# kosmylo/Safe-MARL

Measured on AMD Instinct MI355X. Metric: env-steps/sec (33-bus, 4096 envs/GPU) at 1/2/4/8 MI355X + PF-kernel HBM GB/s, higher is better.
Workload: dtype f64

## Files before the change

safe-marl_amd/csrc/flexenv.hip:

```cpp
#include <hip/hip_runtime.h>
#include <stdint.h>
#include <stdio.h>
#include <string.h>
#include <stdlib.h>
#include <vector>
#include "flex_device.h"
#include "flexnet.h"
#include "actor_r16.h"
#include "agent_sum.h"

#define FLEX_MAX_DEVICES 16
#define HIP_TRY(x) do { hipError_t _e = (x); if (_e != hipSuccess) { \
    fprintf(stderr, "[flexenv] %s failed: %s (%s:%d)\n", #x, hipGetErrorString(_e), __FILE__, __LINE__); \
    return FLEX_EHIP; } } while (0)

enum { AF_E = 0, AF_PRED, AF_CH, AF_DIS, AF_Q, AF_PCT, AF_EINIT, AF_COUNT };
enum { IF_STEPS = 0, IF_START, IF_ROW, IF_OBSCNT, IF_ITERS, IF_SWEEPS, IF_EPISODE, IF_COUNT = 8 };
__host__ __device__ __forceinline__ int agent_rec_doubles(int n_agents) { return (AF_COUNT * n_agents + 7) & ~7; }

struct DevState {
    double* vm;
    uint32_t* vw;
    double* agent;
    double* cumrew;
// ... 172 lines not shown
            const bool live = NA_EXACT || ag < na;
#pragma unroll
            for (int i = 0; i < CLS; ++i) {
                const flex_v2i r = __builtin_amdgcn_raw_buffer_load_b64(rin, live ? src[i] : -1, ag * H3 * 16, 0);
                buf[ag][i] = make_float2(__int_as_float(r.x), __int_as_float(r.y));
            }
        }
    }
    __device__ __forceinline__ void store(const KArgs& a, int env0, bool enable, OutT* __restrict__ out) const {
        const int H = a.cfg.history, na = a.cfg.n_agents, H3 = 3 * H;
        const int env_floats = na * H * 6;
        const int span = enable ? EPW * env_floats : 0;
        const __amdgpu_buffer_rsrc_t rout = __builtin_amdgcn_make_buffer_rsrc(
            (void*)(out + (int64_t)env0 * env_floats), 0, span * (int)sizeof(OutT), FLEX_BUF_FLAGS);
#pragma unroll
        for (int ag = 0; ag < NA_CAP; ++ag) {
            const bool live = NA_EXACT || ag < na;
#pragma unroll
            for (int i = 0; i < CLS; ++i) {
                const int d = live ? dst[i] : -1;
                if constexpr (sizeof(OutT) == 4) {
                    flex_v2i w; w.x = __float_as_int(buf[ag][i].x); w.y = __float_as_int(buf[ag][i].y);
                    __builtin_amdgcn_raw_buffer_store_b64(w, rout, d, ag * H3 * 8, FLEX_AUX_NT);
                } else {
                    const double dx = (double)buf[ag][i].x, dy = (double)buf[ag][i].y;
                    flex_v4i w; w.x = __double2loint(dx); w.y = __double2hiint(dx); w.z = __double2loint(dy); w.w = __double2hiint(dy);
                    __builtin_amdgcn_raw_buffer_store_b128(w, rout, d, ag * H3 * 16, FLEX_AUX_NT);
                }
            }
        }
    }
};

template <int EPW, typename OutT>
__device__ __forceinline__ void obs_store_new(const KArgs& a, int env0, int g, bool valid, const LaneNet& ln, int k,
                                              double pd, double qd, double ppv, double v, double price, double e,
                                              OutT* __restrict__ out, float* __restrict__ rows) {
    const int H = a.cfg.history, na = a.cfg.n_agents;
    const int ring_floats = na * H * 12, env_floats = na * H * 6;
    float* const ring = a.st.ring + (int64_t)env0 * ring_floats;
    const int slot = small_mod(k, H, a.inv_h);
    if (valid && ln.agent >= 0) {
        const float2 r0 = make_float2((float)pd, (float)qd), r1 = make_float2((float)ppv, (float)v);
        const float2 r2 = make_float2((float)price, (float)e);
        const uint32_t ro = (uint32_t)(g * ring_floats + (ln.agent * 2 * H + slot) * 6) * 4, mo = ro + (uint32_t)H * 24;
        st_at2(ring, ro, r0); st_at2(ring, ro + 8, r1); st_at2(ring, ro + 16, r2);
        st_at2(ring, mo, r0); st_at2(ring, mo + 8, r1); st_at2(ring, mo + 16, r2);
        if (rows) {
            typedef float rw_f4 __attribute__((ext_vector_type(4)));
            float* const rb = rows + (int64_t)env0 * (na * FLEX_ROW_W);
            const uint32_t wo = (uint32_t)((g * na + ln.agent) * FLEX_ROW_W) * 4;
            const float older = (float)(k < H - 1 ? k : H - 1);
            st_at<rw_f4>(rb, wo, rw_f4{r0.x, r0.y, r1.x, r1.y});
            st_at<rw_f4>(rb, wo + 16, rw_f4{r2.x, r2.y, older, 0.0f});
        }
        if (out) {
            OutT* const o = out + (int64_t)env0 * env_floats;
            const uint32_t oo = (uint32_t)(g * env_floats + (ln.agent * H + (H - 1)) * 6) * (uint32_t)sizeof(OutT);
            if constexpr (sizeof(OutT) == 4) {
                st_at2(o, oo, r0); st_at2(o, oo + 8, r1); st_at2(o, oo + 16, r2);
            } else {
                st_at<double>(o, oo, pd); st_at<double>(o, oo + 8, qd); st_at<double>(o, oo + 16, ppv);
                st_at<double>(o, oo + 24, v); st_at<double>(o, oo + 32, price); st_at<double>(o, oo + 40, e);
            }
        }
    }
}

template <int EPW>
__device__ __forceinline__ void obs_ring_clear(const KArgs& a, int env, bool valid, const LaneNet& ln) {
    constexpr int LW = FLEX_WAVE / EPW;
    const int H = a.cfg.history, na = a.cfg.n_agents;
    float* ring = a.st.ring + (int64_t)env * na * H * 12;
    const int per_agent = (H - 1) * 6;
    if (valid)
        for (int idx = ln.l; idx < na * per_agent; idx += LW) {
            const int ag = idx / per_agent, rem = idx - ag * per_agent;
            ring[(ag * 2 * H + 1) * 6 + rem] = 0.0f;
        }
}

template <int EPW, typename OutT>
__device__ __forceinline__ void push_and_emit_obs(const KArgs& a, int env, bool valid, const LaneNet& ln, int k,
                                                  double pd, double qd, double ppv, double v, double price,
                                                  double e, OutT* __restrict__ out, float* __restrict__ rows, bool fresh) {
    constexpr int LW = FLEX_WAVE / EPW;
    const int H = a.cfg.history, na = a.cfg.n_agents;
    int32_t* ie = a.st.ienv + (int64_t)env * IF_COUNT;
    const int slot = k % H;
    float* ring = a.st.ring + (int64_t)env * na * H * 12;
    OutT* o = out ? out + (int64_t)env * na * H * 6 : nullptr;
    if (valid && ln.agent >= 0) {
        const double feat[6] = {pd, qd, ppv, v, price, e};
        float* r = ring + (ln.agent * 2 * H + slot) * 6;
#pragma unroll
        for (int t = 0; t < 6; ++t) {
            r[t] = (float)feat[t];
            r[H * 6 + t] = (float)feat[t];
            if (o) o[(ln.agent * H + (H - 1)) * 6 + t] = (OutT)feat[t];
// ... 119 lines not shown
        if (failed) { if (or_failed) { if (!ok) failed[env] = 1; } else failed[env] = ok ? 0 : 1; }
    }
    if (ln.l == FLEX_WAVE / EPW - 1 && valid) a.st.cumrew[env] = 0.0;
    obs_ring_clear<EPW>(a, env, valid, ln);
    if (want_obs) push_and_emit_obs<EPW, ObsT>(a, env, valid, ln, 0, pd, qd, ppv, v, price, e_new, obs, rows, true);
}

template <int EPW, typename ObsT>
__global__ __launch_bounds__(FLEX_WAVE * FLEX_WAVES_PER_BLOCK)
void flex_reset_kernel(KArgs a, const uint8_t* __restrict__ mask, DevResetSpec inj, ObsT* __restrict__ obs,
                       int want_obs, uint8_t* __restrict__ failed) {
    EnvSlot<EPW> slot(a.n_envs);
    if (slot.wave_idle(a.n_envs)) return;
    const bool valid = slot.valid && (!mask || mask[slot.env] != 0);
    if (__ballot(valid) == 0ull) return;
    LaneNet ln;
    load_lane_net<EPW>(a.net, slot.lane, ln);
    flex_reset_body<EPW, ObsT>(a, slot.env, valid, ln, inj, obs, want_obs, nullptr, failed, false);
}


#ifndef FLEX_MANY_CARRY_NET
#define FLEX_MANY_CARRY_NET 1
#endif
#ifndef FLEX_MANY_PREFETCH_ACT
#define FLEX_MANY_PREFETCH_ACT 1
#endif
#ifndef FLEX_MANY_EARLY_HEAD
#define FLEX_MANY_EARLY_HEAD 1
#endif
#ifndef FLEX_MANY_HDR_REGS
#define FLEX_MANY_HDR_REGS 1
#endif
struct StepCarry {
    flex_v4i iv;
    bool have;
    bool have_iv;
    LaneNet ln;
    NetHdrRegs hdr;
    float4 af;
    double2 ad0, ad1;
#ifdef FLEX_MANY_STAMPS
    uint32_t st_prev, st_acc[4];
#endif
    double pd, qd, ppv, price, e_cur, e_init, cum;
    uint32_t vw;
};
template <int EPW, typename ObsT, typename ActT, int NA_CAP, bool SINK, bool ROWS, bool MANY = false>
__device__ __forceinline__ void flex_step_body(const KArgs& a, const int wave, const ActT* __restrict__ actions,
                                               double* __restrict__ reward, uint8_t* __restrict__ done, double* __restrict__ info,
                                               uint8_t* __restrict__ failed, ObsT* __restrict__ obs, int want_obs, int auto_reset,
                                               const int64_t slab, const bool cells, const unsigned long long kbase,
                                               StepCarry* mc = nullptr, const ActT* __restrict__ next_actions = nullptr) {
    constexpr int LW = FLEX_WAVE / EPW;
    const int lane = threadIdx.x & 63;
    const int env0 = wave * EPW;
    if (env0 >= a.n_envs) return;
    float* rowrec = nullptr;
    if constexpr (ROWS) {
        if (a.obs_slabs > 0 && obs) {
            const int64_t p = (slab >= 0 ? slab : *a.obs_cursor) + 1;
            rowrec = reinterpret_cast<float*>(obs) + (p >= a.obs_slabs ? 0 : p) * a.obs_slab_stride;
        }
    }
    const bool valid = env0 + lane / LW < a.n_envs;
    const int g = valid ? lane / LW : 0;
    const int env = env0 + g;
    FLEX_STAMP_RT(5);
    FLEX_STAMP(0);
    const FlexCfg& c = a.cfg;
    int32_t* const b_ienv = a.st.ienv + (int64_t)env0 * IF_COUNT;
    const uint32_t o_ienv = g * (IF_COUNT * 4);
    int4 iv;
    LaneNet ln;
    if constexpr (MANY) {
        if (mc->have || mc->have_iv) iv = int4{mc->iv.x, mc->iv.y, mc->iv.z, mc->iv.w};
        else iv = ld_at<int4>(b_ienv, o_ienv);
#if FLEX_MANY_CARRY_NET
        ln = mc->ln;
#else
        load_lane_net<EPW>(a.net, lane, ln);
#endif
    } else {
        iv = ld_at<int4>(b_ienv, o_ienv);
        load_lane_net<EPW>(a.net, lane, ln);
    }
    ln.pq = ln.pq && valid;
    const int nb = a.n_bus, na = c.n_agents;
    const bool is_bus = ln.bus >= 0, is_bld = ln.agent >= 0;
    const int ag = is_bld ? ln.agent : 0, busi = is_bus ? ln.bus : 0;

    const int arec = agent_rec_doubles(na);
    double* const b_agent = a.st.agent + (int64_t)env0 * arec;
    uint32_t* const b_vw = a.st.vw + (int64_t)env0 * LW;
    const ActT* const b_act = actions + (int64_t)env0 * (na * 4);
    const uint32_t o_agent = (g * arec + ag) * 8;
    const uint32_t o_volt = (g * LW + ln.l) * 4;
    const uint32_t o_bus = busi * 8, o_qbus = (nb + busi) * 8, o_pv = (2 * nb + ag) * 8, o_price = (2 * nb + na) * 8;
    const uint32_t AFB = na * 8;

    const int steps = iv.x, start = iv.y, obs_cnt = iv.w;
    const int rows = (int)a.rows;
    const uint32_t row_off = (uint32_t)clamp_row32(iv.z, rows) * (uint32_t)a.row_bytes;

    const bool from_regs = MANY && mc->have;
    const uint32_t o_act = (g * na + ag) * (4 * (uint32_t)sizeof(ActT));
    ActT av[4];
    if constexpr (MANY && FLEX_MANY_PREFETCH_ACT) {
        if constexpr (sizeof(ActT) == 4) { av[0] = mc->af.x; av[1] = mc->af.y; av[2] = mc->af.z; av[3] = mc->af.w; }
        else { av[0] = mc->ad0.x; av[1] = mc->ad0.y; av[2] = mc->ad1.x; av[3] = mc->ad1.y; }
    } else if constexpr (sizeof(ActT) == 4) {
        const float4 t = ld_at<float4>(b_act, o_act);
        av[0] = t.x; av[1] = t.y; av[2] = t.z; av[3] = t.w;
    } else {
        const double2 t0 = ld_at<double2>(b_act, o_act), t1 = ld_at<double2>(b_act, o_act + 16);
        av[0] = t0.x; av[1] = t0.y; av[2] = t1.x; av[3] = t1.y;
    }
    double pd_r, qd_r, ppv_r, price, e_cur_r, e_init_r, cum_before;
    uint32_t vw_word;
    if (from_regs) {
        pd_r = mc->pd; qd_r = mc->qd; ppv_r = mc->ppv; price = mc->price;
        e_cur_r = mc->e_cur; e_init_r = mc->e_init; cum_before = mc->cum; vw_word = mc->vw;
    } else {
        pd_r = ld_at<double>(a.series, row_off + o_bus); qd_r = ld_at<double>(a.series, row_off + o_qbus);
        ppv_r = ld_at<double>(a.series, row_off + o_pv); price = ld_at<double>(a.series, row_off + o_price);
        e_cur_r = ld_at<double>(b_agent, o_agent + AF_E * AFB);
        e_init_r = ld_at<double>(b_agent, o_agent + AF_EINIT * AFB);
        vw_word = ld_at<uint32_t>(b_vw, o_volt);
        cum_before = ld_at<double>(a.st.cumrew + env0, g * 8);
    }
    double we, wf;
    unpack_warm(vw_word, we, wf);
    const int new_row = clamp_row32(start + steps, rows);
    const uint32_t nrow_off = (uint32_t)new_row * (uint32_t)a.row_bytes;
    if constexpr (MANY && FLEX_MANY_PREFETCH_ACT) {
        const ActT* const b_nact = next_actions + (int64_t)env0 * (na * 4);
        if constexpr (sizeof(ActT) == 4) mc->af = ld_at<float4>(b_nact, o_act);
        else { mc->ad0 = ld_at<double2>(b_nact, o_act); mc->ad1 = ld_at<double2>(b_nact, o_act + 16); }
    }
    double n_pd = ld_at<double>(a.series, nrow_off + (is_bld || MANY ? o_bus : o_price));
    double n_qd = ld_at<double>(a.series, nrow_off + (is_bld || MANY ? o_qbus : o_price));
    double n_ppv = ld_at<double>(a.series, nrow_off + (is_bld || MANY ? o_pv : o_price));
    const double n_price = ld_at<double>(a.series, nrow_off + o_price);
    const bool obs_fast = want_obs && (ROWS || (na <= NA_CAP && 3 * c.history <= FLEX_OBS_CLASSES(EPW) * LW));
    ObsHist<EPW, ROWS ? 1 : NA_CAP, ObsT> hist;
    if constexpr (!ROWS) hist.load(a, env0, g, valid, obs_fast, ln, obs_cnt);

    const bool warm = c.warm_start != 0 && ln.pq;
    double e = warm ? we : 1.0, f = warm ? wf : 0.0;

    const double pd = is_bus ? pd_r : 0.0, qd = is_bus ? qd_r : 0.0, ppv = is_bld ? ppv_r : 0.0;
    const double e_cur = is_bld ? e_cur_r : 0.0, e_init = is_bld ? (steps == 1 ? e_init_r : e_cur_r) : 0.0;
    FlexAct act = parse_actions(c, a.inv_eta_ch, a.inv_eta_dis, c.raw_actions != 0, (double)av[0], (double)av[1],
                                (double)av[2], (double)av[3], pd, ppv, e_cur);
    if (!is_bld) { act.pct = 0.0; act.pred = 0.0; act.ch = 0.0; act.dis = 0.0; act.q = 0.0; }
    const double pnet = pd - act.pred - ppv + act.ch - act.dis;
    const double qnet = qd - act.q;
    typedef float sk_f4 __attribute__((ext_vector_type(4)));
    sk_f4 sk_hv[SINK ? 3 : 1];
    float sk_av = 0.0f;
    int64_t sk_p = 0;
    if constexpr (SINK) {
        sk_p = slab >= 0 ? slab : *a.obs_cursor;
        const FlexReplaySink& sk = a.sink;
        const sk_f4* hs = reinterpret_cast<const sk_f4*>(sk.hid_new + (int64_t)env * sk.hid_w);
        const int h4 = sk.hid_w >> 2;
#pragma unroll
        for (int r = 0; r < 3; ++r) { const int i = ln.l + LW * r; sk_hv[r] = hs[i < h4 ? i : 0]; }
        sk_av = sk.policy_action[(int64_t)env * sk.act_w + (ln.l < sk.act_w ? ln.l : 0)];
    }

    int iters = 0, sweeps = 0;
#ifdef FLEX_STAMPS
    asm volatile("" :: "v"(pnet), "v"(qnet), "v"(e), "v"(f));
    asm volatile("s_waitcnt vmcnt(0)" ::: "memory");
#endif
    FLEX_STAMP(1);
#ifdef FLEX_MANY_STAMPS
    if constexpr (MANY) { asm volatile("" :: "v"(pnet), "v"(qnet), "v"(e), "v"(f)); FLEX_MANY_STAMP(mc, 0); }
#endif
    bool ok;
    if constexpr (MANY && FLEX_MANY_HDR_REGS)
        ok = pf_solve<EPW>(mc->hdr, a.net, ln, c.solver, pnet, qnet, e, f, c.pf_tol, c.pf_max_iter, iters, sweeps);
    else
        ok = pf_solve<EPW>(a.net, ln, c.solver, pnet, qnet, e, f, c.pf_tol, c.pf_max_iter, iters, sweeps);
#ifdef FLEX_STAMPS
    asm volatile("" :: "v"(e), "v"(f));
#endif
    FLEX_STAMP(2);
#ifdef FLEX_MANY_STAMPS
    if constexpr (MANY) { asm volatile("" :: "v"(e), "v"(f)); FLEX_MANY_STAMP(mc, 1); }
#endif

    const KArgs& z = *relaunder_kernarg<KArgs>(kbase);
    const FlexCfg& cz = z.cfg;
    if constexpr (!ROWS) hist.store(z, env0, obs_fast, obs);
    double* const e_agent = z.st.agent + (int64_t)env0 * agent_rec_doubles(cz.n_agents);
    uint32_t* const e_vw = z.st.vw + (int64_t)env0 * LW;
    {
        bool wave_dom;
        const bool dom_bad = grp_any<EPW>(is_bld && valid && e_init + cz.dt * (cz.eta_ch * act.ch - z.inv_eta_dis * act.dis) < -FLEX_DOMAIN_EPS,
                                          ln.grp, wave_dom);
        ok = ok && !dom_bad;
    }
    double* const e_vm = z.st.vm + (int64_t)env0 * z.n_bus;
    int32_t* const e_ienv = z.st.ienv + (int64_t)env0 * IF_COUNT;
    const uint32_t o_vm = (g * z.n_bus + busi) * 8;
    double v, pred, ch, dis, q, e_new;
    if (ok) {
        v = sqrt(e * e + f * f);
        pred = act.pred; ch = act.ch; dis = act.dis; q = act.q;
        e_new = e_init + cz.dt * (cz.eta_ch * ch - z.inv_eta_dis * dis);
        if (ln.pq) {
            st_at<double>(e_vm, o_vm, v);
            st_at<uint32_t>(e_vw, o_volt, pack_warm(e, f));
        }
        if (is_bld && valid) {
            st_at<double>(e_agent, o_agent + AF_PRED * AFB, pred);
            st_at<double>(e_agent, o_agent + AF_CH * AFB, ch);
            st_at<double>(e_agent, o_agent + AF_DIS * AFB, dis);
            st_at<double>(e_agent, o_agent + AF_Q * AFB, q);
        }
    } else {
        v = is_bus ? ld_at<double>(e_vm, o_vm) : 1.0;
        pred = is_bld ? ld_at<double>(e_agent, o_agent + AF_PRED * AFB) : 0.0;
        ch = is_bld ? ld_at<double>(e_agent, o_agent + AF_CH * AFB) : 0.0;
        dis = is_bld ? ld_at<double>(e_agent, o_agent + AF_DIS * AFB) : 0.0;
        q = is_bld ? ld_at<double>(e_agent, o_agent + AF_Q * AFB) : 0.0;
        e_new = e_cur;
    }
    if (is_bld && valid) {
        st_at<double>(e_agent, o_agent + AF_PCT * AFB, act.pct);
        st_at<double>(e_agent, o_agent + AF_E * AFB, e_new);
    }

    RewardOut rw = reward_terms<EPW>(cz, ln, is_bld, price, pred, ch, dis, q, v);
    double* const b_cum = z.st.cumrew + env0;
    double rwd = rw.reward;
    if (!ok) rwd -= cz.fail_penalty;
    const int new_steps = steps + 1;
    const bool term = (new_steps >= cz.episode_limit) || !ok;
    const bool restart = auto_reset && term && valid;
    if (ln.l == LW - 1 && valid) {
        st_at<double>(reward + env0, g * 8, rwd);
        if (info) {
            double* const io = info + (int64_t)env0 * FLEX_INFO_W;
            const uint32_t oi = g * (FLEX_INFO_W * 8);
            st_at<double>(io, oi, rw.reward); st_at<double>(io, oi + 8, rw.revenue); st_at<double>(io, oi + 16, rw.der);
            st_at<double>(io, oi + 24, rw.ess); st_at<double>(io, oi + 32, rw.disc); st_at<double>(io, oi + 40, rw.vpen);
            st_at<double>(io, oi + 48, cum_before);
        }
        st_at<double>(b_cum, g * 8, cum_before + rwd);
    }
    const int cnt_after = obs_cnt + ((want_obs && obs_fast && !restart) ? 1 : 0);
    if constexpr (MANY) {
        mc->iv = flex_v4i{new_steps, start, new_row, cnt_after};
        mc->have = !(auto_reset && __ballot(restart) != 0ull);
        mc->have_iv = false;
        mc->pd = n_pd; mc->qd = n_qd; mc->ppv = n_ppv; mc->price = n_price;
        mc->e_cur = e_new; mc->e_init = e_init_r; mc->cum = cum_before + rwd;
        mc->vw = (ok && ln.bus >= 0) ? pack_warm(e, f) : vw_word;
    }
    if (ln.l == 0 && valid) {
        done[env] = term ? 1 : 0;
        if (failed) failed[env] = ok ? 0 : 1;
        st_at<flex_v4i>(e_ienv, o_ienv, flex_v4i{new_steps, start, new_row, cnt_after});
        st_at<flex_v2i>(e_ienv, o_ienv + IF_ITERS * 4, flex_v2i{iters, sweeps});
    }
    if constexpr (SINK) {
        const KArgs& zs = *relaunder_kernarg<KArgs>(kbase);
        const FlexReplaySink& sk = zs.sink;
        const int64_t p = sk_p;
        const int64_t pn = p + 1 >= zs.obs_slabs ? 0 : p + 1;
        const float keep = term ? 0.0f : 1.0f;
        if (valid) {
            sk_f4* hd = reinterpret_cast<sk_f4*>(sk.hid_ring + (pn * zs.n_envs + env) * (int64_t)sk.hid_w);
            const int h4 = sk.hid_w >> 2;
            float* const sm = sk.small_ring + (p * zs.n_envs + env) * (int64_t)sk.small_w;
#pragma unroll
            for (int r = 0; r < 3; ++r) { const int i = ln.l + LW * r; if (i < h4) hd[i] = sk_hv[r] * keep; }
            if (ln.l < sk.act_w) sm[ln.l] = sk_av;
            if (ln.l == LW - 1) {
                const int na_ = cz.n_agents;
                for (int j = 0; j < na_; ++j) sm[sk.act_w + j] = (float)rwd;
                sm[sk.act_w + na_] = 1.0f - keep;
                sm[sk.act_w + na_ + 1] = 1.0f - keep;
                double* const ac = sk.acc + (int64_t)env * 10;
                unsafeAtomicAdd(ac + 0, rw.reward); unsafeAtomicAdd(ac + 1, rw.revenue); unsafeAtomicAdd(ac + 2, rw.der);
                unsafeAtomicAdd(ac + 3, rw.ess); unsafeAtomicAdd(ac + 4, rw.disc); unsafeAtomicAdd(ac + 5, rw.vpen);
                unsafeAtomicAdd(ac + 6, cum_before); unsafeAtomicAdd(ac + 7, rwd); unsafeAtomicAdd(ac + 8, ok ? 0.0 : 1.0);
            }
        }
        if (cells && blockIdx.x == 0 && threadIdx.x == 0) {
            if (sk.cursor_out) *sk.cursor_out = pn;
            if (sk.aux_counter) *sk.aux_counter += 1;
        }
    }
#ifdef FLEX_STAMPS
    asm volatile("s_waitcnt vmcnt(0)" ::: "memory");
#endif
    FLEX_STAMP(3);
    if (want_obs) {
        n_pd = is_bld ? n_pd : 0.0; n_qd = is_bld ? n_qd : 0.0; n_ppv = is_bld ? n_ppv : 0.0;
        const bool emit = valid && !restart;
        ObsT* const out = ROWS ? nullptr : obs;
        if (obs_fast) obs_store_new<EPW, ObsT>(z, env0, g, emit, ln, obs_cnt, n_pd, n_qd, n_ppv, v, n_price, e_new, out, rowrec);
        else push_and_emit_obs<EPW, ObsT>(z, env, emit, ln, obs_cnt, n_pd, n_qd, n_ppv, v, n_price, e_new, out, rowrec, false);
    }
    if (auto_reset && __ballot(restart) != 0ull) {
        LaneNet ln0;
        if constexpr (MANY && FLEX_MANY_CARRY_NET) ln0 = mc->ln;
        else load_lane_net<EPW>(a.net, lane, ln0);
        const DevResetSpec none = {nullptr, nullptr, nullptr, nullptr, nullptr};
        const KArgs& ar = *relaunder_kernarg<KArgs>(kbase);
        flex_reset_body<EPW, ObsT>(ar, env, restart, ln0, none, ROWS ? nullptr : obs, want_obs, rowrec, failed, true);
    }
    if (cells && blockIdx.x == 0 && threadIdx.x == 0) {
        const KArgs* const ac = relaunder_kernarg<KArgs>(kbase);
        int64_t* const sc = ac->step_counter;
        if (sc) {
            const int64_t nx = *sc + 1;
            *sc = (ac->step_modulo > 0 && nx >= ac->step_modulo) ? 0 : nx;
        }
    }
#ifdef FLEX_STAMPS
    asm volatile("s_waitcnt vmcnt(0)" ::: "memory");
#endif
    FLEX_STAMP(4);
    FLEX_STAMP_RT(6);
}

template <int EPW, typename ObsT, typename ActT, int NA_CAP, bool SINK = false, bool ROWS = false>
__global__ __launch_bounds__(FLEX_WAVE * FLEX_WAVES_PER_BLOCK, 8 / FLEX_WAVES_PER_BLOCK)
void flex_step_kernel(KArgs a, const ActT* __restrict__ actions, double* __restrict__ reward,
                      uint8_t* __restrict__ done, double* __restrict__ info, uint8_t* __restrict__ failed,
                      ObsT* __restrict__ obs, int want_obs, int auto_reset) {
    const int wave = __builtin_amdgcn_readfirstlane(blockIdx.x * FLEX_WAVES_PER_BLOCK + (threadIdx.x >> 6));
    flex_step_body<EPW, ObsT, ActT, NA_CAP, SINK, ROWS>(a, wave, actions, reward, done, info, failed, obs, want_obs, auto_reset, -1, true,
                                                  (unsigned long long)__builtin_amdgcn_kernarg_segment_ptr());
}

struct ManyArgs {
    KArgs k;
    const void* actions;
    double* reward;
    uint8_t* done;
    double* info;
    uint8_t* failed;
    int32_t n_steps, act_period, auto_reset, carry;
};

template <int EPW, typename ActT>
__global__ __launch_bounds__(FLEX_WAVE * FLEX_WAVES_PER_BLOCK, 8 / FLEX_WAVES_PER_BLOCK)
void flex_step_many_kernel(ManyArgs m) {
    const unsigned long long kb = (unsigned long long)__builtin_amdgcn_kernarg_segment_ptr();
    const int wave = __builtin_amdgcn_readfirstlane(blockIdx.x * FLEX_WAVES_PER_BLOCK + (threadIdx.x >> 6));
    if (wave * EPW >= m.k.n_envs) return;
    StepCarry mc;
    mc.have = false;
    mc.have_iv = false;
    mc.iv = flex_v4i{0, 0, 0, 0};
    const int lane = threadIdx.x & 63;
#if FLEX_MANY_EARLY_HEAD || FLEX_MANY_PREFETCH_ACT
    constexpr int LW = FLEX_WAVE / EPW;
    const int g0 = wave * EPW + lane / LW < m.k.n_envs ? lane / LW : 0;
#endif
#if FLEX_MANY_EARLY_HEAD
    mc.iv = ld_at<flex_v4i>(m.k.st.ienv + (int64_t)wave * EPW * IF_COUNT, g0 * (IF_COUNT * 4));
    mc.have_iv = true;
#endif
#if FLEX_MANY_PREFETCH_ACT
    const int agent0 = m.k.net->agent_of_lane[lane & (LW - 1)];
#endif
    load_lane_net<EPW>(m.k.net, lane, mc.ln);
#if FLEX_MANY_PREFETCH_ACT
    {
        const int na = m.k.cfg.n_agents;
        const ActT* const b_act = reinterpret_cast<const ActT*>(m.actions) + (int64_t)wave * EPW * (na * 4);
        const uint32_t o_act = (g0 * na + (agent0 >= 0 ? agent0 : 0)) * (4 * (uint32_t)sizeof(ActT));
        if constexpr (sizeof(ActT) == 4) mc.af = ld_at<float4>(b_act, o_act);
        else { mc.ad0 = ld_at<double2>(b_act, o_act); mc.ad1 = ld_at<double2>(b_act, o_act + 16); }
    }
#endif
#if FLEX_MANY_HDR_REGS
    mc.hdr = load_net_hdr(m.k.net);
#endif
#ifdef FLEX_MANY_STAMPS
    mc.st_acc[0] = mc.st_acc[1] = mc.st_acc[2] = mc.st_acc[3] = 0;
    uint32_t st_first[4] = {0, 0, 0, 0};
    FLEX_MANY_STAMP(&mc, -1);
    const uint32_t st_begin = mc.st_prev;
#endif
    const int n_steps = m.n_steps;
    const bool carry = m.carry != 0;
    int slot = 0;
    for (int k = 0; k < n_steps; ++k) {
        const ManyArgs& b = *relaunder_kernarg<ManyArgs>(kb);
        const int64_t ne = b.k.n_envs;
        const int64_t slab_elems = ne * (b.k.cfg.n_agents * 4);
        const ActT* act = reinterpret_cast<const ActT*>(b.actions) + (int64_t)slot * slab_elems;
        slot = slot + 1 == b.act_period ? 0 : slot + 1;
        const ActT* act_next = reinterpret_cast<const ActT*>(b.actions) + (int64_t)slot * slab_elems;
        if (!carry) mc.have = false;
        flex_step_body<EPW, float, ActT, FLEX_OBS_AGENTS_SMALL, false, true, true>(
            b.k, wave, act, b.reward + k * ne, b.done + k * ne, b.info ? b.info + k * ne * FLEX_INFO_W : nullptr,
            b.failed ? b.failed + k * ne : nullptr, nullptr, 1, b.auto_reset, -1, false, kb, &mc, act_next);
        FLEX_MANY_STAMP(&mc, 2);
        __builtin_amdgcn_fence(__ATOMIC_RELEASE, "workgroup");
        __builtin_amdgcn_fence(__ATOMIC_ACQUIRE, "workgroup");
        FLEX_MANY_STAMP(&mc, 3);
#ifdef FLEX_MANY_STAMPS
        if (k == 0) {
#pragma unroll
            for (int i = 0; i < 4; ++i) { st_first[i] = mc.st_acc[i]; mc.st_acc[i] = 0; }
        }
#endif
    }
#ifdef FLEX_MANY_STAMPS
    if (m.k.stamps && lane == 0) {
        unsigned long long* const o = m.k.stamps + (int64_t)wave * EPW * 16;
#pragma unroll
        for (int i = 0; i < 4; ++i) { o[i] = st_first[i]; o[4 + i] = mc.st_acc[i]; }
        o[8] = (unsigned long long)n_steps;
        o[9] = mc.st_prev - st_begin;
    }
#endif
    if (blockIdx.x == 0 && threadIdx.x == 0) {
        const ManyArgs& b = *relaunder_kernarg<ManyArgs>(kb);
        int64_t* const sc = b.k.step_counter;
        if (sc) {
            int64_t nx = *sc + n_steps;
            if (b.k.step_modulo > 0) nx %= b.k.step_modulo;
            *sc = nx;
        }
    }
}


template <int EPW, typename ObsT>
__global__ __launch_bounds__(FLEX_WAVE * FLEX_WAVES_PER_BLOCK)
void flex_obs_kernel(KArgs a, ObsT* __restrict__ obs) {
    EnvSlot<EPW> slot(a.n_envs);
    if (slot.wave_idle(a.n_envs)) return;
// ... 855 lines not shown
        HIP_TRY(hipGetLastError());
        return FLEX_OK;
    }
    const bool f64 = obs && obs_dtype == FLEX_F64;
    const int want = obs ? 1 : 0;
#define FLEX_LAUNCH_STEP(EPW_, OBS_, ACT_) do { \
        if (small_obs) hipLaunchKernelGGL((flex_step_kernel<EPW_, OBS_, ACT_, FLEX_OBS_AGENTS_SMALL>), grid, env_block(), 0, s, k, \
            (const ACT_*)actions, reward, done, info, failed, (OBS_*)obs, want, auto_reset); \
        else hipLaunchKernelGGL((flex_step_kernel<EPW_, OBS_, ACT_, FLEX_OBS_AGENTS_LARGE>), grid, env_block(), 0, s, k, \
            (const ACT_*)actions, reward, done, info, failed, (OBS_*)obs, want, auto_reset); } while (0)
    const bool small_obs = e->cfg.n_agents == FLEX_OBS_AGENTS_SMALL && 3 * e->cfg.history <= FLEX_OBS_CLASSES(epw) * (FLEX_WAVE / epw);
    const int variant = (epw == 2 ? 4 : 0) + (f64 ? 2 : 0) + (act_dtype == FLEX_F64 ? 1 : 0);
    switch (variant) {
        case 0: FLEX_LAUNCH_STEP(1, float, float); break;
        case 1: FLEX_LAUNCH_STEP(1, float, double); break;
        case 2: FLEX_LAUNCH_STEP(1, double, float); break;
        case 3: FLEX_LAUNCH_STEP(1, double, double); break;
        case 4: FLEX_LAUNCH_STEP(2, float, float); break;
        case 5: FLEX_LAUNCH_STEP(2, float, double); break;
        case 6: FLEX_LAUNCH_STEP(2, double, float); break;
        default: FLEX_LAUNCH_STEP(2, double, double); break;
    }
#undef FLEX_LAUNCH_STEP
    HIP_TRY(hipGetLastError());
    return FLEX_OK;
}

int flexenv_step_many(FlexEnv* e, const void* actions, int32_t act_dtype, int32_t act_period, int32_t steps,
                      double* reward, uint8_t* done, double* info, uint8_t* failed, int32_t flags, void* stream) {
    if (!e || !actions || !reward || !done || steps < 1 || act_period < 1) return FLEX_EINVAL;
    if (act_dtype != FLEX_F32 && act_dtype != FLEX_F64) return FLEX_EINVAL;
    if (flags & ~(FLEX_STEP_AUTORESET | FLEX_STEP_OBS_ROWS | FLEX_STEP_MANY_NO_CARRY)) return FLEX_EINVAL;
    if (!(flags & FLEX_STEP_OBS_ROWS) || e->obs_slabs > 0) return FLEX_EINVAL;
    ManyArgs m;
    m.k = make_args(e);
    m.k.step_counter = e->step_counter; m.k.step_modulo = e->step_modulo;
    m.actions = actions; m.reward = reward; m.done = done; m.info = info; m.failed = failed;
    m.n_steps = steps; m.act_period = act_period; m.auto_reset = (flags & FLEX_STEP_AUTORESET) ? 1 : 0;
    m.carry = (flags & FLEX_STEP_MANY_NO_CARRY) ? 0 : 1;
    hipStream_t s = (hipStream_t)stream;
    const int epw = e->hnet.epw;
    const dim3 grid = env_grid(e->n_envs, epw);
    if (epw == 2 && act_dtype == FLEX_F32) hipLaunchKernelGGL((flex_step_many_kernel<2, float>), grid, env_block(), 0, s, m);
    else if (epw == 2) hipLaunchKernelGGL((flex_step_many_kernel<2, double>), grid, env_block(), 0, s, m);
    else if (act_dtype == FLEX_F32) hipLaunchKernelGGL((flex_step_many_kernel<1, float>), grid, env_block(), 0, s, m);
    else hipLaunchKernelGGL((flex_step_many_kernel<1, double>), grid, env_block(), 0, s, m);
    HIP_TRY(hipGetLastError());
    return FLEX_OK;
}

static bool burst_config_ok(const FlexEnv* e, const FlexActorArgs* actor, const double* reward, const uint8_t* done,
                            const float* obs_ring, int32_t steps, bool mlp = false) {
    if (!e || !actor || !reward || !done || !obs_ring || steps < 1) return false;
    const FlexActorArgs& p = *actor;
    const int na = e->cfg.n_agents;
    if (!e->has_sink || e->obs_slabs < 2 || e->hnet.epw != 2 || na > 5) return false;
    if (p.rows != (int64_t)e->n_envs * na || p.n_agents != na || p.obs_dim < 1 || p.obs_dim > FLEXNET_MAX_OBS || (p.obs_dim & 3) ||
        p.act_dim < 1 || p.act_dim > FLEXNET_MAX_ACT) return false;
    if (!mlp && (!p.hidden_in || !p.w_ih || !p.w_hh || !p.b_ih || !p.b_hh)) return false;
    if (!p.hidden_out || !p.means || !p.action || !p.env_action || !p.cursor || !p.cursor_out ||
        !p.fc1_w || !p.fc1_b || !p.fc2_w || !p.fc2_b ||
        (p.layernorm && (!p.ln_w || !p.ln_b))) return false;
    if (p.ring_slabs != e->obs_slabs || steps >= e->obs_slabs || p.obs_dim != 6 * e->cfg.history) return false;
    if (p.cursor_out != e->obs_cursor || p.cursor != e->sink.cursor_out || p.hidden_out != e->sink.hid_new ||
        p.action != e->sink.policy_action) return false;
    return !p.save_z1;
}

static BurstArgs burst_args(FlexEnv* e, const FlexActorArgs& p, double* reward, uint8_t* done, double* info, uint8_t* failed,
                            float* obs_ring, int32_t steps) {
    BurstArgs b;
    b.k = make_args(e);
// ... 457 lines not shown
```

Baseline: 658.5 million.

## Pack per-phase kernel constants into cache-line blocks for multi-step kernel

```diff
diff --git a/safe-marl_amd/csrc/flexenv.hip b/safe-marl_amd/csrc/flexenv.hip
--- a/safe-marl_amd/csrc/flexenv.hip
+++ b/safe-marl_amd/csrc/flexenv.hip
@@ -228,14 +228,28 @@
     }
 };
 
-template <int EPW, typename OutT>
-__device__ __forceinline__ void obs_store_new(const KArgs& a, int env0, int g, bool valid, const LaneNet& ln, int k,
-                                              double pd, double qd, double ppv, double v, double price, double e,
-                                              OutT* __restrict__ out, float* __restrict__ rows) {
-    const int H = a.cfg.history, na = a.cfg.n_agents;
+struct ObsSrcArgs {
+    const KArgs& a;
+    __device__ __forceinline__ int history() const { return a.cfg.history; }
+    __device__ __forceinline__ int n_agents() const { return a.cfg.n_agents; }
+    __device__ __forceinline__ float* ring_at(int env0, int ring_floats) const { return a.st.ring + (int64_t)env0 * ring_floats; }
+    __device__ __forceinline__ float inv_h() const { return a.inv_h; }
+};
+struct ObsSrcHeld {
+    float* ring; int H, na; float inv;
+    __device__ __forceinline__ int history() const { return H; }
+    __device__ __forceinline__ int n_agents() const { return na; }
+    __device__ __forceinline__ float* ring_at(int, int) const { return ring; }
+    __device__ __forceinline__ float inv_h() const { return inv; }
+};
+template <int EPW, typename OutT, typename Src>
+__device__ __forceinline__ void obs_store_new_from(const Src& a, int env0, int g, bool valid, const LaneNet& ln, int k,
+                                                   double pd, double qd, double ppv, double v, double price, double e,
+                                                   OutT* __restrict__ out, float* __restrict__ rows) {
+    const int H = a.history(), na = a.n_agents();
     const int ring_floats = na * H * 12, env_floats = na * H * 6;
-    float* const ring = a.st.ring + (int64_t)env0 * ring_floats;
-    const int slot = small_mod(k, H, a.inv_h);
+    float* const ring = a.ring_at(env0, ring_floats);
+    const int slot = small_mod(k, H, a.inv_h());
     if (valid && ln.agent >= 0) {
         const float2 r0 = make_float2((float)pd, (float)qd), r1 = make_float2((float)ppv, (float)v);
         const float2 r2 = make_float2((float)price, (float)e);
@@ -261,6 +275,12 @@
             }
         }
     }
+}
+template <int EPW, typename OutT>
+__device__ __forceinline__ void obs_store_new(const KArgs& a, int env0, int g, bool valid, const LaneNet& ln, int k,
+                                              double pd, double qd, double ppv, double v, double price, double e,
+                                              OutT* __restrict__ out, float* __restrict__ rows) {
+    obs_store_new_from<EPW, OutT>(ObsSrcArgs{a}, env0, g, valid, ln, k, pd, qd, ppv, v, price, e, out, rows);
 }
 
 template <int EPW>
@@ -446,12 +466,58 @@
 #ifndef FLEX_MANY_HDR_REGS
 #define FLEX_MANY_HDR_REGS 1
 #endif
+#ifndef FLEX_MANY_CONSTS
+#define FLEX_MANY_CONSTS 1
+#endif
+__host__ __device__ constexpr bool many_consts(int epw) { return FLEX_MANY_CONSTS != 0 && epw == 2; }
+struct alignas(64) ManyConstsP {
+    const double* series;
+    const DevNet* net;
+    double pf_tol, e_max, e_min;
+    int32_t n_envs, na_nb;
+    int32_t rows, row_bytes;
+    int32_t flags;
+    int32_t pf_max_iter;
+    double max_power_reduction, p_ch_max, p_dis_max, tan_phi, eta_ch, eta_dis, inv_eta_ch, inv_eta_dis;
+    const char* actions;
+    int64_t act_stride;
+    int32_t act_env_bytes;
+    int32_t act_period;
+};
+struct alignas(64) ManyConstsE {
+    double dt, eta_ch, inv_eta_dis, v_max, v_min, pv_cost, ess_cost, discomfort_coeff;
+    double voltage_coeff, fail_penalty;
+    double* reward; uint8_t* done; double* info; uint8_t* failed;
+    int32_t n_envs;
+    int32_t episode_limit;
+    int32_t cfgw;
+    float inv_h;
+};
+struct ManyConsts { ManyConstsP p; ManyConstsE e; };
+static_assert(sizeof(ManyConstsP) == 192 && sizeof(ManyConstsE) == 128, "whole 64-byte lines per phase");
+struct ManyArgs {
+    KArgs k;
+    const void* actions;
+    double* reward;
+    uint8_t* done;
+    double* info;
+    uint8_t* failed;
+    int32_t n_steps, act_period, auto_reset, carry;
+    ManyConsts c;
+};
+struct ManyWave {
+    double* agent; uint32_t* vw; double* vm; int32_t* ienv; double* cumrew; float* ring;
+    int64_t row;
+    int32_t slot;
+};
 struct StepCarry {
     flex_v4i iv;
     bool have;
     bool have_iv;
     LaneNet ln;
     NetHdrRegs hdr;
+    ManyWave w;
+    ManyConstsP P;
     float4 af;
     double2 ad0, ad1;
 #ifdef FLEX_MANY_STAMPS
@@ -467,9 +533,13 @@
                                                const int64_t slab, const bool cells, const unsigned long long kbase,
                                                StepCarry* mc = nullptr, const ActT* __restrict__ next_actions = nullptr) {
     constexpr int LW = FLEX_WAVE / EPW;
+    constexpr bool MC = MANY && many_consts(EPW);
+    static_assert(!MC || (ROWS && !SINK), "the launch of many steps pushes rows and files into no sink");
     const int lane = threadIdx.x & 63;
     const int env0 = wave * EPW;
-    if (env0 >= a.n_envs) return;
+    ManyConstsP P;
+    if constexpr (MC) P = mc->P;
+    if (env0 >= (MC ? P.n_envs : a.n_envs)) return;
     float* rowrec = nullptr;
     if constexpr (ROWS) {
         if (a.obs_slabs > 0 && obs) {
@@ -477,13 +547,21 @@
             rowrec = reinterpret_cast<float*>(obs) + (p >= a.obs_slabs ? 0 : p) * a.obs_slab_stride;
         }
     }
-    const bool valid = env0 + lane / LW < a.n_envs;
+    const bool valid = env0 + lane / LW < (MC ? P.n_envs : a.n_envs);
     const int g = valid ? lane / LW : 0;
     const int env = env0 + g;
     FLEX_STAMP_RT(5);
     FLEX_STAMP(0);
-    const FlexCfg& c = a.cfg;
-    int32_t* const b_ienv = a.st.ienv + (int64_t)env0 * IF_COUNT;
+    FlexCfg pc;
+    if constexpr (MC) {
+        pc.max_power_reduction = P.max_power_reduction; pc.p_ch_max = P.p_ch_max; pc.p_dis_max = P.p_dis_max; pc.tan_phi = P.tan_phi;
+        pc.eta_ch = P.eta_ch; pc.eta_dis = P.eta_dis; pc.e_max = P.e_max; pc.e_min = P.e_min;
+    }
+    const FlexCfg* const cp = MC ? &pc : &a.cfg;
+    const FlexCfg& c = *cp;
+    int32_t* b_ienv;
+    if constexpr (MC) b_ienv = mc->w.ienv;
+    else b_ienv = a.st.ienv + (int64_t)env0 * IF_COUNT;
     const uint32_t o_ienv = g * (IF_COUNT * 4);
     int4 iv;
     LaneNet ln;
@@ -500,22 +578,35 @@
         load_lane_net<EPW>(a.net, lane, ln);
     }
     ln.pq = ln.pq && valid;
-    const int nb = a.n_bus, na = c.n_agents;
+    const int nb = MC ? P.na_nb >> 16 : a.n_bus, na = MC ? P.na_nb & 0xffff : c.n_agents;
     const bool is_bus = ln.bus >= 0, is_bld = ln.agent >= 0;
     const int ag = is_bld ? ln.agent : 0, busi = is_bus ? ln.bus : 0;
 
     const int arec = agent_rec_doubles(na);
-    double* const b_agent = a.st.agent + (int64_t)env0 * arec;
-    uint32_t* const b_vw = a.st.vw + (int64_t)env0 * LW;
-    const ActT* const b_act = actions + (int64_t)env0 * (na * 4);
+    double* b_agent;
+    uint32_t* b_vw;
+    const ActT* b_act;
+    int32_t nslot = 0;
+    if constexpr (MC) {
+        b_agent = mc->w.agent; b_vw = mc->w.vw;
+        b_act = reinterpret_cast<const ActT*>(P.actions + mc->w.slot * P.act_stride + (int64_t)env0 * P.act_env_bytes);
+        nslot = mc->w.slot + 1 == P.act_period ? 0 : mc->w.slot + 1;
+        mc->w.slot = nslot;
+    } else {
+        b_agent = a.st.agent + (int64_t)env0 * arec;
+        b_vw = a.st.vw + (int64_t)env0 * LW;
+        b_act = actions + (int64_t)env0 * (na * 4);
+    }
+    const auto series = [&]() -> const double* { if constexpr (MC) return P.series; else return a.series; };
+    const auto row_bytes = [&]() -> uint32_t { if constexpr (MC) return (uint32_t)P.row_bytes; else return (uint32_t)a.row_bytes; };
     const uint32_t o_agent = (g * arec + ag) * 8;
     const uint32_t o_volt = (g * LW + ln.l) * 4;
     const uint32_t o_bus = busi * 8, o_qbus = (nb + busi) * 8, o_pv = (2 * nb + ag) * 8, o_price = (2 * nb + na) * 8;
     const uint32_t AFB = na * 8;
 
     const int steps = iv.x, start = iv.y, obs_cnt = iv.w;
-    const int rows = (int)a.rows;
-    const uint32_t row_off = (uint32_t)clamp_row32(iv.z, rows) * (uint32_t)a.row_bytes;
+    const int rows = MC ? P.rows : (int)a.rows;
+    const uint32_t row_off = (uint32_t)clamp_row32(iv.z, rows) * row_bytes();
 
     const bool from_regs = MANY && mc->have;
     const uint32_t o_act = (g * na + ag) * (4 * (uint32_t)sizeof(ActT));
@@ -536,36 +627,41 @@
         pd_r = mc->pd; qd_r = mc->qd; ppv_r = mc->ppv; price = mc->price;
         e_cur_r = mc->e_cur; e_init_r = mc->e_init; cum_before = mc->cum; vw_word = mc->vw;
     } else {
-        pd_r = ld_at<double>(a.series, row_off + o_bus); qd_r = ld_at<double>(a.series, row_off + o_qbus);
-        ppv_r = ld_at<double>(a.series, row_off + o_pv); price = ld_at<double>(a.series, row_off + o_price);
+        pd_r = ld_at<double>(series(), row_off + o_bus); qd_r = ld_at<double>(series(), row_off + o_qbus);
+        ppv_r = ld_at<double>(series(), row_off + o_pv); price = ld_at<double>(series(), row_off + o_price);
         e_cur_r = ld_at<double>(b_agent, o_agent + AF_E * AFB);
         e_init_r = ld_at<double>(b_agent, o_agent + AF_EINIT * AFB);
         vw_word = ld_at<uint32_t>(b_vw, o_volt);
-        cum_before = ld_at<double>(a.st.cumrew + env0, g * 8);
+        if constexpr (MC) cum_before = ld_at<double>(mc->w.cumrew, g * 8);
+        else cum_before = ld_at<double>(a.st.cumrew + env0, g * 8);
     }
     double we, wf;
     unpack_warm(vw_word, we, wf);
     const int new_row = clamp_row32(start + steps, rows);
-    const uint32_t nrow_off = (uint32_t)new_row * (uint32_t)a.row_bytes;
+    const uint32_t nrow_off = (uint32_t)new_row * row_bytes();
     if constexpr (MANY && FLEX_MANY_PREFETCH_ACT) {
-        const ActT* const b_nact = next_actions + (int64_t)env0 * (na * 4);
+        const ActT* b_nact;
+        if constexpr (MC) {
+            b_nact = reinterpret_cast<const ActT*>(P.actions + nslot * P.act_stride + (int64_t)env0 * P.act_env_bytes);
+        } else b_nact = next_actions + (int64_t)env0 * (na * 4);
         if constexpr (sizeof(ActT) == 4) mc->af = ld_at<float4>(b_nact, o_act);
         else { mc->ad0 = ld_at<double2>(b_nact, o_act); mc->ad1 = ld_at<double2>(b_nact, o_act + 16); }
     }
-    double n_pd = ld_at<double>(a.series, nrow_off + (is_bld || MANY ? o_bus : o_price));
-    double n_qd = ld_at<double>(a.series, nrow_off + (is_bld || MANY ? o_qbus : o_price));
-    double n_ppv = ld_at<double>(a.series, nrow_off + (is_bld || MANY ? o_pv : o_price));
-    const double n_price = ld_at<double>(a.series, nrow_off + o_price);
+    double n_pd = ld_at<double>(series(), nrow_off + (is_bld || MANY ? o_bus : o_price));
+    double n_qd = ld_at<double>(series(), nrow_off + (is_bld || MANY ? o_qbus : o_price));
+    double n_ppv = ld_at<double>(series(), nrow_off + (is_bld || MANY ? o_pv : o_price));
+    const double n_price = ld_at<double>(series(), nrow_off + o_price);
     const bool obs_fast = want_obs && (ROWS || (na <= NA_CAP && 3 * c.history <= FLEX_OBS_CLASSES(EPW) * LW));
     ObsHist<EPW, ROWS ? 1 : NA_CAP, ObsT> hist;
     if constexpr (!ROWS) hist.load(a, env0, g, valid, obs_fast, ln, obs_cnt);
 
-    const bool warm = c.warm_start != 0 && ln.pq;
+    const bool warm = (MC ? (P.flags & 2) != 0 : c.warm_start != 0) && ln.pq;
     double e = warm ? we : 1.0, f = warm ? wf : 0.0;
 
     const double pd = is_bus ? pd_r : 0.0, qd = is_bus ? qd_r : 0.0, ppv = is_bld ? ppv_r : 0.0;
     const double e_cur = is_bld ? e_cur_r : 0.0, e_init = is_bld ? (steps == 1 ? e_init_r : e_cur_r) : 0.0;
-    FlexAct act = parse_actions(c, a.inv_eta_ch, a.inv_eta_dis, c.raw_actions != 0, (double)av[0], (double)av[1],
+    FlexAct act = parse_actions(c, MC ? P.inv_eta_ch : a.inv_eta_ch, MC ? P.inv_eta_dis : a.inv_eta_dis,
+                                MC ? (P.flags & 1) != 0 : c.raw_actions != 0, (double)av[0], (double)av[1],
                                 (double)av[2], (double)av[3], pd, ppv, e_cur);
     if (!is_bld) { act.pct = 0.0; act.pred = 0.0; act.ch = 0.0; act.dis = 0.0; act.q = 0.0; }
     const double pnet = pd - act.pred - ppv + act.ch - act.dis;
@@ -594,7 +690,11 @@
     if constexpr (MANY) { asm volatile("" :: "v"(pnet), "v"(qnet), "v"(e), "v"(f)); FLEX_MANY_STAMP(mc, 0); }
 #endif
     bool ok;
-    if constexpr (MANY && FLEX_MANY_HDR_REGS)
+    if constexpr (MC && FLEX_MANY_HDR_REGS)
+        ok = pf_solve<EPW>(mc->hdr, P.net, ln, P.flags >> 8, pnet, qnet, e, f, P.pf_tol, P.pf_max_iter, iters, sweeps);
+    else if constexpr (MC)
+        ok = pf_solve<EPW>(P.net, ln, P.flags >> 8, pnet, qnet, e, f, P.pf_tol, P.pf_max_iter, iters, sweeps);
+    else if constexpr (MANY && FLEX_MANY_HDR_REGS)
         ok = pf_solve<EPW>(mc->hdr, a.net, ln, c.solver, pnet, qnet, e, f, c.pf_tol, c.pf_max_iter, iters, sweeps);
     else
         ok = pf_solve<EPW>(a.net, ln, c.solver, pnet, qnet, e, f, c.pf_tol, c.pf_max_iter, iters, sweeps);
@@ -607,24 +707,42 @@
 #endif
 
     const KArgs& z = *relaunder_kernarg<KArgs>(kbase);
-    const FlexCfg& cz = z.cfg;
+    ManyConstsE E;
+    FlexCfg ec;
+    if constexpr (MC) {
+        E = relaunder_kernarg<ManyArgs>(kbase)->c.e;
+        ec.dt = E.dt; ec.eta_ch = E.eta_ch; ec.v_max = E.v_max; ec.v_min = E.v_min; ec.pv_cost = E.pv_cost; ec.ess_cost = E.ess_cost;
+        ec.discomfort_coeff = E.discomfort_coeff; ec.voltage_coeff = E.voltage_coeff; ec.fail_penalty = E.fail_penalty;
+        ec.episode_limit = E.episode_limit; ec.history = (int)((uint32_t)E.cfgw >> 16); ec.n_agents = E.cfgw & 0xff;
+        auto_reset = (E.cfgw >> 15) & 1;
+    }
+    const FlexCfg* const czp = MC ? &ec : &z.cfg;
+    const FlexCfg& cz = *czp;
     if constexpr (!ROWS) hist.store(z, env0, obs_fast, obs);
-    double* const e_agent = z.st.agent + (int64_t)env0 * agent_rec_doubles(cz.n_agents);
-    uint32_t* const e_vw = z.st.vw + (int64_t)env0 * LW;
+    double* e_agent;
+    uint32_t* e_vw;
+    if constexpr (MC) {
+        e_agent = mc->w.agent; e_vw = mc->w.vw;
+    } else {
+        e_agent = z.st.agent + (int64_t)env0 * agent_rec_doubles(cz.n_agents);
+        e_vw = z.st.vw + (int64_t)env0 * LW;
+    }
     {
         bool wave_dom;
-        const bool dom_bad = grp_any<EPW>(is_bld && valid && e_init + cz.dt * (cz.eta_ch * act.ch - z.inv_eta_dis * act.dis) < -FLEX_DOMAIN_EPS,
+        const bool dom_bad = grp_any<EPW>(is_bld && valid && e_init + cz.dt * (cz.eta_ch * act.ch - (MC ? E.inv_eta_dis : z.inv_eta_dis) * act.dis) < -FLEX_DOMAIN_EPS,
                                           ln.grp, wave_dom);
         ok = ok && !dom_bad;
     }
-    double* const e_vm = z.st.vm + (int64_t)env0 * z.n_bus;
-    int32_t* const e_ienv = z.st.ienv + (int64_t)env0 * IF_COUNT;
-    const uint32_t o_vm = (g * z.n_bus + busi) * 8;
+    double* e_vm;
+    int32_t* e_ienv;
+    if constexpr (MC) { e_vm = mc->w.vm; e_ienv = mc->w.ienv; }
+    else { e_vm = z.st.vm + (int64_t)env0 * z.n_bus; e_ienv = z.st.ienv + (int64_t)env0 * IF_COUNT; }
+    const uint32_t o_vm = (g * (MC ? (E.cfgw >> 8) & 0x7f : z.n_bus) + busi) * 8;
     double v, pred, ch, dis, q, e_new;
     if (ok) {
         v = sqrt(e * e + f * f);
         pred = act.pred; ch = act.ch; dis = act.dis; q = act.q;
-        e_new = e_init + cz.dt * (cz.eta_ch * ch - z.inv_eta_dis * dis);
+        e_new = e_init + cz.dt * (cz.eta_ch * ch - (MC ? E.inv_eta_dis : z.inv_eta_dis) * dis);
         if (ln.pq) {
             st_at<double>(e_vm, o_vm, v);
             st_at<uint32_t>(e_vw, o_volt, pack_warm(e, f));
@@ -649,16 +767,25 @@
     }
 
     RewardOut rw = reward_terms<EPW>(cz, ln, is_bld, price, pred, ch, dis, q, v);
-    double* const b_cum = z.st.cumrew + env0;
+    double* b_cum;
+    double* b_rew;
+    double* b_info;
+    if constexpr (MC) {
+        const int64_t row = mc->w.row;
+        b_cum = mc->w.cumrew; b_rew = E.reward + (row + env0); b_info = E.info ? E.info + (row + env0) * FLEX_INFO_W : nullptr;
+        done = E.done + row; failed = E.failed ? E.failed + row : nullptr;
+    } else {
+        b_cum = z.st.cumrew + env0; b_rew = reward + env0; b_info = info;
+    }
     double rwd = rw.reward;
     if (!ok) rwd -= cz.fail_penalty;
     const int new_steps = steps + 1;
     const bool term = (new_steps >= cz.episode_limit) || !ok;
     const bool restart = auto_reset && term && valid;
     if (ln.l == LW - 1 && valid) {
-        st_at<double>(reward + env0, g * 8, rwd);
-        if (info) {
-            double* const io = info + (int64_t)env0 * FLEX_INFO_W;
+        st_at<double>(b_rew, g * 8, rwd);
+        if (b_info) {
+            double* const io = MC ? b_info : b_info + (int64_t)env0 * FLEX_INFO_W;
             const uint32_t oi = g * (FLEX_INFO_W * 8);
             st_at<double>(io, oi, rw.reward); st_at<double>(io, oi + 8, rw.revenue); st_at<double>(io, oi + 16, rw.der);
             st_at<double>(io, oi + 24, rw.ess); st_at<double>(io, oi + 32, rw.disc); st_at<double>(io, oi + 40, rw.vpen);
@@ -718,8 +845,14 @@
         n_pd = is_bld ? n_pd : 0.0; n_qd = is_bld ? n_qd : 0.0; n_ppv = is_bld ? n_ppv : 0.0;
         const bool emit = valid && !restart;
         ObsT* const out = ROWS ? nullptr : obs;
-        if (obs_fast) obs_store_new<EPW, ObsT>(z, env0, g, emit, ln, obs_cnt, n_pd, n_qd, n_ppv, v, n_price, e_new, out, rowrec);
+        if constexpr (MC)
+            obs_store_new_from<EPW, ObsT>(ObsSrcHeld{mc->w.ring, cz.history, cz.n_agents, E.inv_h}, env0, g, emit, ln, obs_cnt,
+                                          n_pd, n_qd, n_ppv, v, n_price, e_new, out, rowrec);
+        else if (obs_fast) obs_store_new<EPW, ObsT>(z, env0, g, emit, ln, obs_cnt, n_pd, n_qd, n_ppv, v, n_price, e_new, out, rowrec);
         else push_and_emit_obs<EPW, ObsT>(z, env, emit, ln, obs_cnt, n_pd, n_qd, n_ppv, v, n_price, e_new, out, rowrec, false);
+    }
+    if constexpr (MC) {
+        mc->w.row += E.n_envs;
     }
     if (auto_reset && __ballot(restart) != 0ull) {
         LaneNet ln0;
@@ -753,16 +886,6 @@
     flex_step_body<EPW, ObsT, ActT, NA_CAP, SINK, ROWS>(a, wave, actions, reward, done, info, failed, obs, want_obs, auto_reset, -1, true,
                                                   (unsigned long long)__builtin_amdgcn_kernarg_segment_ptr());
 }
-
-struct ManyArgs {
-    KArgs k;
-    const void* actions;
-    double* reward;
-    uint8_t* done;
-    double* info;
-    uint8_t* failed;
-    int32_t n_steps, act_period, auto_reset, carry;
-};
 
 template <int EPW, typename ActT>
 __global__ __launch_bounds__(FLEX_WAVE * FLEX_WAVES_PER_BLOCK, 8 / FLEX_WAVES_PER_BLOCK)
@@ -807,22 +930,43 @@
 #endif
     const int n_steps = m.n_steps;
     const bool carry = m.carry != 0;
+    if constexpr (many_consts(EPW)) {
+        const int64_t e0 = (int64_t)wave * EPW;
+        const int na = m.k.cfg.n_agents;
+        ManyWave& w = mc.w;
+        w.agent = m.k.st.agent + e0 * agent_rec_doubles(na);
+        w.vw = m.k.st.vw + e0 * (FLEX_WAVE / EPW);
+        w.vm = m.k.st.vm + e0 * m.k.n_bus;
+        w.ienv = m.k.st.ienv + e0 * IF_COUNT;
+        w.cumrew = m.k.st.cumrew + e0;
+        w.ring = m.k.st.ring + e0 * (na * m.k.cfg.history * 12);
+        w.row = 0;
+        w.slot = 0;
+        mc.P = relaunder_kernarg<ManyArgs>(kb)->c.p;
+    }
     int slot = 0;
     for (int k = 0; k < n_steps; ++k) {
         const ManyArgs& b = *relaunder_kernarg<ManyArgs>(kb);
-        const int64_t ne = b.k.n_envs;
-        const int64_t slab_elems = ne * (b.k.cfg.n_agents * 4);
-        const ActT* act = reinterpret_cast<const ActT*>(b.actions) + (int64_t)slot * slab_elems;
-        slot = slot + 1 == b.act_period ? 0 : slot + 1;
-        const ActT* act_next = reinterpret_cast<const ActT*>(b.actions) + (int64_t)slot * slab_elems;
-        if (!carry) mc.have = false;
-        flex_step_body<EPW, float, ActT, FLEX_OBS_AGENTS_SMALL, false, true, true>(
-            b.k, wave, act, b.reward + k * ne, b.done + k * ne, b.info ? b.info + k * ne * FLEX_INFO_W : nullptr,
-            b.failed ? b.failed + k * ne : nullptr, nullptr, 1, b.auto_reset, -1, false, kb, &mc, act_next);
+        if constexpr (many_consts(EPW)) {
+            if (!carry) mc.have = false;
+            flex_step_body<EPW, float, ActT, FLEX_OBS_AGENTS_SMALL, false, true, true>(
+                b.k, wave, nullptr, nullptr, nullptr, nullptr, nullptr, nullptr, 1, 0, -1, false, kb, &mc, nullptr);
+        } else {
+            const int64_t ne = b.k.n_envs;
+            const int64_t slab_elems = ne * (b.k.cfg.n_agents * 4);
+            const ActT* act = reinterpret_cast<const ActT*>(b.actions) + (int64_t)slot * slab_elems;
+            slot = slot + 1 == b.act_period ? 0 : slot + 1;
+            const ActT* act_next = reinterpret_cast<const ActT*>(b.actions) + (int64_t)slot * slab_elems;
+            if (!carry) mc.have = false;
+            flex_step_body<EPW, float, ActT, FLEX_OBS_AGENTS_SMALL, false, true, true>(
+                b.k, wave, act, b.reward + k * ne, b.done + k * ne, b.info ? b.info + k * ne * FLEX_INFO_W : nullptr,
+                b.failed ? b.failed + k * ne : nullptr, nullptr, 1, b.auto_reset, -1, false, kb, &mc, act_next);
+        }
         FLEX_MANY_STAMP(&mc, 2);
         __builtin_amdgcn_fence(__ATOMIC_RELEASE, "workgroup");
         __builtin_amdgcn_fence(__ATOMIC_ACQUIRE, "workgroup");
         FLEX_MANY_STAMP(&mc, 3);
+        if constexpr (many_consts(EPW)) mc.P = relaunder_kernarg<ManyArgs>(kb)->c.p;
 #ifdef FLEX_MANY_STAMPS
         if (k == 0) {
 #pragma unroll
@@ -1744,12 +1888,37 @@
     if (act_dtype != FLEX_F32 && act_dtype != FLEX_F64) return FLEX_EINVAL;
     if (flags & ~(FLEX_STEP_AUTORESET | FLEX_STEP_OBS_ROWS | FLEX_STEP_MANY_NO_CARRY)) return FLEX_EINVAL;
     if (!(flags & FLEX_STEP_OBS_ROWS) || e->obs_slabs > 0) return FLEX_EINVAL;
+    if (e->cfg.history >= 32768) return FLEX_EINVAL;
     ManyArgs m;
     m.k = make_args(e);
     m.k.step_counter = e->step_counter; m.k.step_modulo = e->step_modulo;
     m.actions = actions; m.reward = reward; m.done = done; m.info = info; m.failed = failed;
     m.n_steps = steps; m.act_period = act_period; m.auto_reset = (flags & FLEX_STEP_AUTORESET) ? 1 : 0;
     m.carry = (flags & FLEX_STEP_MANY_NO_CARRY) ? 0 : 1;
+    {
+        const FlexCfg& c = m.k.cfg;
+        memset(&m.c, 0, sizeof(m.c));
+        ManyConstsP& p = m.c.p;
+        p.series = m.k.series; p.net = m.k.net;
+        p.pf_tol = c.pf_tol; p.e_max = c.e_max; p.e_min = c.e_min;
+        p.n_envs = m.k.n_envs; p.na_nb = c.n_agents | (m.k.n_bus << 16);
+        p.rows = (int32_t)m.k.rows; p.row_bytes = m.k.row_bytes;
+        p.flags = (c.raw_actions != 0 ? 1 : 0) | (c.warm_start != 0 ? 2 : 0) | (c.solver << 8);
+        p.pf_max_iter = c.pf_max_iter;
+        p.max_power_reduction = c.max_power_reduction; p.p_ch_max = c.p_ch_max; p.p_dis_max = c.p_dis_max; p.tan_phi = c.tan_phi;
+        p.eta_ch = c.eta_ch; p.eta_dis = c.eta_dis; p.inv_eta_ch = m.k.inv_eta_ch; p.inv_eta_dis = m.k.inv_eta_dis;
+        p.actions = (const char*)actions;
+        p.act_env_bytes = c.n_agents * 4 * (act_dtype == FLEX_F32 ? 4 : 8);
+        p.act_stride = (int64_t)m.k.n_envs * p.act_env_bytes;
+        p.act_period = act_period;
+        ManyConstsE& q = m.c.e;
+        q.dt = c.dt; q.eta_ch = c.eta_ch; q.inv_eta_dis = m.k.inv_eta_dis; q.v_max = c.v_max; q.v_min = c.v_min;
+        q.pv_cost = c.pv_cost; q.ess_cost = c.ess_cost; q.discomfort_coeff = c.discomfort_coeff; q.voltage_coeff = c.voltage_coeff;
+        q.fail_penalty = c.fail_penalty;
+        q.reward = reward; q.done = done; q.info = info; q.failed = failed;
+        q.n_envs = m.k.n_envs; q.episode_limit = c.episode_limit; q.inv_h = m.k.inv_h;
+        q.cfgw = (int32_t)((uint32_t)c.n_agents | (uint32_t)m.k.n_bus << 8 | (uint32_t)m.auto_reset << 15 | (uint32_t)c.history << 16);
+    }
     hipStream_t s = (hipStream_t)stream;
     const int epw = e->hnet.epw;
     const dim3 grid = env_grid(e->n_envs, epw);
```

Measured after the change: 669.4 million, median of 6. +1.6%, better.
